# matteosantama/dantzig

Hardware: AMD Instinct MI355X
Metric: simplex_iterations_per_sec (higher is better)
Workload: dtype f64

## Files before the change

dantzig_amd/_build.py:

```python
from __future__ import annotations

import os
import shutil
import subprocess
from concurrent.futures import ThreadPoolExecutor

HERE = os.path.dirname(os.path.abspath(__file__))
CSRC = os.path.join(HERE, "csrc")
OBJ = os.path.join(HERE, "_obj")
LIB = os.path.join(HERE, "libdantzig_amd.so")
ARCH = "gfx950"
SOURCES = ["engine.hip", "k_vector.hip", "k_price.hip", "k_strict.hip", "k_fast.hip", "k_chain.hip", "k_sparse.hip", "k_refactor.hip", "k_rowshard.hip", "k_drift.hip", "k_batch.hip", "k_batch_fast.hip",
           "k_mip.hip", "k_duals.hip", "k_ranging.hip", "k_rays.hip", "model.cpp", "mip.cpp", "lpgen.cpp"]
FLAGS = ["-O3", "-std=c++17", "-fPIC", "-ffp-contract=off", "-fno-fast-math", "-Wall",
         "-Wno-unused-result", "-Wno-unused-value"]


def _hipcc() -> str:
    exe = shutil.which("hipcc") or "/opt/rocm/bin/hipcc"
    if not os.path.exists(exe):
        raise RuntimeError("hipcc not found: dantzig_amd needs the ROCm toolchain to build")
    return exe


def _newest(paths) -> float:
    return max(os.path.getmtime(p) for p in paths)


def _deps():
    hdrs = [os.path.join(CSRC, "common.h"), os.path.join(CSRC, "k_price_kernels.h"),
            os.path.join(CSRC, "fast_decide.h"), os.path.join(CSRC, "fast_rows.h"),
            os.path.join(CSRC, "chain_barrier.h"), os.path.join(CSRC, "batch_strict.h"),
            os.path.join(CSRC, "batch_host.h"),
            os.path.join(CSRC, "mip_internal.h"), os.path.join(CSRC, "duals.h"), os.path.join(CSRC, "ranging.h"), os.path.join(CSRC, "rays.h"),
            os.path.join(os.path.dirname(HERE), "include", "dantzig_amd.h")]
    return hdrs


def _compile(src: str) -> str:
    path = os.path.join(CSRC, src)
    obj = os.path.join(OBJ, src + ".o")
    if os.path.exists(obj) and os.path.getmtime(obj) >= _newest([path] + _deps()):
        return obj
    cmd = [_hipcc(), f"--offload-arch={ARCH}", *FLAGS, "-c", path, "-o", obj]
    if src.endswith(".cpp"):
        cmd.insert(1, "-x")
        cmd.insert(2, "c++")
        cmd = [c for c in cmd if not c.startswith("--offload-arch")]
    subprocess.check_call(cmd)
    return obj


def build(force: bool = False, verbose: bool = False) -> str:
    os.makedirs(OBJ, exist_ok=True)
    if force:
# ... 17 lines not shown
```

dantzig_amd/csrc/chain_barrier.h:

```cpp
#pragma once
#include "common.h"

#define CH_THREADS 512
#define CH_AGCAP DZG_CHAIN_AGCAP
#define CH_GROUPS 8
#define CH_PAD 16

__device__ __forceinline__ void st_sc1(double *p, double v)
{
    __hip_atomic_store(p, v, __ATOMIC_RELAXED, __HIP_MEMORY_SCOPE_AGENT);
}
__device__ __forceinline__ void st_sc1(int *p, int v)
{
    __hip_atomic_store(p, v, __ATOMIC_RELAXED, __HIP_MEMORY_SCOPE_AGENT);
}
__device__ __forceinline__ double ld_sc1(const double *p)
{
    return __hip_atomic_load(p, __ATOMIC_RELAXED, __HIP_MEMORY_SCOPE_AGENT);
}
__device__ __forceinline__ int ld_sc1(const int *p)
{
    return __hip_atomic_load(p, __ATOMIC_RELAXED, __HIP_MEMORY_SCOPE_AGENT);
}

#define CH_BAR_WORDS (CH_PAD * (2 + CH_GROUPS))
#define CH_POISON (1ull << 62)

__device__ __forceinline__ bool chain_barrier(DzgCtl *ctl, unsigned long long *bar,
                                              unsigned long long &gen)
{
    __shared__ int s_bar_ok;
    __syncthreads();
    if (threadIdx.x == 0) {
        gen += 1;
        const unsigned grp = blockIdx.x % CH_GROUPS;
        const unsigned long long members = (gridDim.x - grp + CH_GROUPS - 1) / CH_GROUPS;
        const unsigned long long ngroups = gridDim.x < CH_GROUPS ? gridDim.x : CH_GROUPS;
        const unsigned long long target = gen * ngroups;
        unsigned long long *frozen = bar + (size_t)CH_PAD * (1 + CH_GROUPS);
        __builtin_amdgcn_s_waitcnt(0);
        const unsigned long long old = __hip_atomic_fetch_add(
            bar + (size_t)CH_PAD * (1 + grp), 1ull, __ATOMIC_RELAXED, __HIP_MEMORY_SCOPE_AGENT);
        int ok = -1;
        unsigned long long val = 0;
        if (old + 1 == gen * members) {
            val = __hip_atomic_fetch_add(bar, 1ull, __ATOMIC_RELAXED, __HIP_MEMORY_SCOPE_AGENT);
            if (val & CH_POISON) ok = 0;
            val = 0;
        }
        if (ok < 0) {
            int spin = 0;
            for (; spin < (1 << 24); ++spin) {
                val = __hip_atomic_load(bar, __ATOMIC_RELAXED, __HIP_MEMORY_SCOPE_AGENT);
                if (val >= target) break;
                __builtin_amdgcn_s_sleep(1);
            }
            if (spin == (1 << 24)) {
                val = __hip_atomic_fetch_or(bar, CH_POISON, __ATOMIC_RELAXED, __HIP_MEMORY_SCOPE_AGENT);
                if (!(val & CH_POISON)) {
                    __hip_atomic_store(frozen, val + 1, __ATOMIC_RELAXED, __HIP_MEMORY_SCOPE_AGENT);
                    ok = val >= target ? 1 : 0;
                }
            } else if (!(val & CH_POISON)) {
                ok = 1;
            }
        }
        if (ok < 0) {
            unsigned long long f = 0;
            for (int spin = 0; spin < (1 << 22) && f == 0; ++spin) {
                f = __hip_atomic_load(frozen, __ATOMIC_RELAXED, __HIP_MEMORY_SCOPE_AGENT);
                if (f == 0) __builtin_amdgcn_s_sleep(1);
            }
            ok = (f != 0 && f - 1 >= target) ? 1 : 0;
        }
        if (!ok) {
            __hip_atomic_store(&ctl->status, (int)DZG_PANIC, __ATOMIC_RELAXED, __HIP_MEMORY_SCOPE_AGENT);
            __hip_atomic_store(&ctl->bar_timeout, 1, __ATOMIC_RELAXED, __HIP_MEMORY_SCOPE_AGENT);
        }
        s_bar_ok = ok;
    }
    __syncthreads();
    return s_bar_ok != 0;
}
```

dantzig_amd/csrc/common.h:

```cpp
#pragma once

#include <hip/hip_runtime.h>
#include <stdint.h>

#include "../../include/dantzig_amd.h"

#define DZG_WAVE 64

struct DzgCtl {
    int status;
    int kind;
    long long iter;
    long long iter_stop;
    int enter_pos;
    int leave_pos;
    int enter_var;
    int leave_var;
    double mu;
    double t, s, tbar, sbar;
    long long nb_struct;
    double price_bytes;
    int lu_mu;
    int lu_pivot_zero;
    int ncompact;
// ... 476 lines not shown
    const double *A;
    int csc;
    const long long *cptr;
    const int *ridx;
    const double *cval;
    const int *var_col;
    int *basis, *nonbasis;
    double *x, *xbar, *z, *zbar;
    double *dx, *dz, *v, *acol;
    DzgCtl *ctl;
    int *log_kind, *log_enter, *log_leave;
    double *log_mu;
    long long log_cap;
    double *binv;
    long long ldb;
    int *drow;
    int *dslot;
    double *U;
    double *W;
    long long ldw;
    double *Wc;
    double *ag;
    double *beta;
    double *beta_part;
    int beta_split;
    int *plist;
    int *pslot;
    int *pcode;
    int *cpos;
    double *fpx_r, *fpz_r, *rx_r, *rz_r;
    int *fpx_k, *fpz_k, *rx_k, *rz_k;
    double *fpx_h, *fpz_h, *rx_h, *rz_h;
    double *log_margin;
    int *bcode, *nbcode;
    int spb;
    const long long *rptr;
    const int *cidx;
    const double *rval;
    int *sslot;
    int *spos;
    int *bslot;
    int *rowpos;
    int *bcnt;
    int *bcol;
    double *bval;
    double *dxs;
    int *acol_code;
    int *lcnt;
// ... 129 lines not shown
```

dantzig_amd/csrc/engine.hip:

```cpp
#include <dlfcn.h>

#include <chrono>
#include <cstdio>
#include <cstdlib>
#include <cstring>
#include <limits>
#include <string>
#include <utility>
#include <algorithm>
#include <vector>

#include "common.h"
#include "duals.h"
#include "ranging.h"
#include "rays.h"

static thread_local std::string g_err;

static int fail(int code, const std::string &msg)
{
    g_err = msg;
    return code;
}

// ... 330 lines not shown
    if (o.stream) {
        s->st = (hipStream_t)o.stream;
        s->own_stream = false;
    } else {
        HIP_OK(hipStreamCreate(&s->st));
    }
    HIP_OK(hipHostMalloc((void **)&s->h_ctl, sizeof(DzgCtl)));

    DzgDev &d = s->d;
    const int m = (int)lp->m, n = (int)lp->n, ns = (int)lp->n_struct, q = n - m;
    d.m = m; d.n = n; d.ns = ns; d.q = q;
    d.lda = ((long long)m + 15) / 16 * 16 + (m >= 2048 ? 272 : 0);
    if (d.lda == 0) d.lda = 16;
    d.eps = o.epsilon;
    d.ftran_variant = -1;
    if (const char *fv = std::getenv("DZG_FTRAN_VARIANT")) d.ftran_variant = std::atoi(fv);
    {
        const double kk = 384e6 / (8.0 * (double)(lp->m > 0 ? lp->m : 1));
        d.ftran_nt_k = kk > 2e9 ? 2000000000 : (int)kk;
        if (d.ftran_nt_k < 513) d.ftran_nt_k = 513;
    }
    d.beta_split = 1;
    if (const char *bs = std::getenv("DZG_CHAIN_BETA_SPLIT")) d.beta_split = bs[0] != '0';
    d.fold_k = 0x7fffffff;
    if (const char *fk = std::getenv("DZG_CHAIN_FOLD_K")) d.fold_k = std::atoi(fk);
    d.world = o.world > 1 ? o.world : 1;
    d.rank = d.world > 1 ? o.rank : 0;
    d.col0 = 0;
    d.col1 = ns;
    if (d.world > 1) {
        if (o.rank < 0 || o.rank >= o.world || o.col_begin < 0 || o.col_end > ns ||
            o.col_begin > o.col_end)
            return fail(DZG_E_ARG, "opts.rank / col_begin / col_end");
        d.col0 = (int)o.col_begin;
        d.col1 = (int)o.col_end;
    }
    const int nloc = d.col1 - d.col0;
    d.repl = (d.world > 1 && o.replicate_matrix && lp->a) ? 1 : 0;
    d.xstride = d.repl ? 8 : 8 + ((long long)m + 7) / 8 * 8;
    const double *a_host = !lp->a ? nullptr
                           : (o.a_is_block && d.world > 1) ? lp->a
                                                           : lp->a + (size_t)d.col0 * (size_t)lp->lda;

    d.csc = (ns > 0 && !lp->a) ? 1 : 0;
    d.rs = 0;
    d.rs_r0 = 0;
// ... 229 lines not shown
            HIP_OK(hipMemcpyAsync(s->dr_c, lp->c, sizeof(double) * n, hipMemcpyHostToDevice, s->st));
            HIP_OK(hipMemcpyAsync(s->dr_cb, cbar.data(), sizeof(double) * n, hipMemcpyHostToDevice, s->st));
            HIP_OK(hipStreamSynchronize(s->st));
        }
        {
            const long long base = ((long long)m + 15) / 16 * 16;
            long long pad = ((160 - base % 512) % 512 + 512) % 512;
            if (pad < 32) pad += 512;
            if (const char *e = std::getenv("DZG_LDB_PAD")) pad = std::atoi(e) / 16 * 16;
            d.ldb = base + pad;
        }
        d.ldw = ((long long)m + 15) / 16 * 16 + 64;
        {
            const size_t rows_kept = d.rs ? (size_t)(d.rs_r1 - d.rs_r0) : (size_t)m;
            double *binv_alloc = nullptr;
            TRY(dev_alloc(s, &binv_alloc, (rows_kept ? rows_kept : 1) * (size_t)d.ldb));
            d.binv = binv_alloc - (d.rs ? (long long)d.rs_r0 * d.ldb : 0);
        }
        TRY(dev_alloc(s, &d.drow, (size_t)m)); TRY(dev_alloc(s, &d.dslot, (size_t)m));
        TRY(dev_alloc(s, &d.U, (size_t)d.ldw * DZG_RMAX));
        TRY(dev_alloc(s, &d.W, (size_t)d.ldw * DZG_RMAX));
        TRY(dev_alloc(s, &d.Wc, (size_t)d.ldw * DZG_RMAX));
        TRY(dev_alloc(s, &d.ag, (size_t)m + 2)); TRY(dev_alloc(s, &d.beta, (size_t)DZG_RMAX));
        TRY(dev_alloc(s, &d.beta_part, (size_t)4 * DZG_RMAX));
        TRY(dev_alloc(s, &d.plist, (size_t)q)); TRY(dev_alloc(s, &d.pslot, (size_t)q));
        TRY(dev_alloc(s, &d.bcode, (size_t)m)); TRY(dev_alloc(s, &d.nbcode, (size_t)q));
        TRY(dev_alloc(s, &d.pcode, (size_t)q));
        if (!d.csc) TRY(dev_alloc(s, &d.cpos, (size_t)(d.col1 > d.col0 ? d.col1 - d.col0 : 1)));
        const size_t np = 4096;
        TRY(dev_alloc(s, &d.fpx_r, np)); TRY(dev_alloc(s, &d.fpz_r, np));
        TRY(dev_alloc(s, &d.rx_r, np)); TRY(dev_alloc(s, &d.rz_r, np));
        TRY(dev_alloc(s, &d.fpx_k, np)); TRY(dev_alloc(s, &d.fpz_k, np));
        TRY(dev_alloc(s, &d.rx_k, np)); TRY(dev_alloc(s, &d.rz_k, np));
        TRY(dev_alloc(s, &d.fpx_h, np)); TRY(dev_alloc(s, &d.fpz_h, np));
        TRY(dev_alloc(s, &d.rx_h, np)); TRY(dev_alloc(s, &d.rz_h, np));
        if (o.refactor_interval != 0) TRY(refactor_workspace(s));
        if (d.spb && !o.seven_launches) {
            hipDeviceProp_t prop;
            HIP_OK(hipGetDeviceProperties(&prop, o.device));
            const int cus = prop.multiProcessorCount > 0 ? prop.multiProcessorCount : 1;
            const char *off = std::getenv("DZG_SP_FUSED");
            if (!(off && off[0] == '0') && (long long)dzg_sp_fused_resident_per_cu() * cus >= dzg_sp_grid(m)) {
                TRY(dev_alloc(s, &s->chain_bar, (size_t)DZG_CHAIN_BAR_WORDS));
                HIP_OK(hipMemsetAsync(s->chain_bar, 0, sizeof(unsigned long long) * DZG_CHAIN_BAR_WORDS, s->st));
            }
        }
        if (d.spb) {
// ... 529 lines not shown
    }
    default: return health_give_up(s, stop);
    }
}

static int budget_spent(dzg_solver *s, bool *spent)
{
    *spent = s->h_ctl->status == DZG_RUNNING && s->h_ctl->iter >= s->h_ctl->iter_stop;
    if (*spent) {
        int st = DZG_ITER_LIMIT;
        HIP_OK(hipMemcpy(&s->d.ctl->status, &st, sizeof(int), hipMemcpyHostToDevice));
        s->h_ctl->status = st;
    }
    return 0;
}

static int chain_recover(dzg_solver *s)
{
    DzgCtl *h = s->h_ctl;
    s->chain_fallbacks += 1;
    s->chain_retry_iter = s->chain_fallbacks >= 3 ? std::numeric_limits<long long>::max()
                                                  : h->iter + 64ll * s->opts.poll_interval;
    HIP_OK(hipMemsetAsync(s->chain_bar, 0, sizeof(unsigned long long) * DZG_CHAIN_BAR_WORDS, s->st));
    h->status = DZG_RUNNING;
    h->bar_timeout = 0;
    h->bar_gen = 0;
    HIP_OK(hipMemcpyAsync(&s->d.ctl->status, &h->status, sizeof(int), hipMemcpyHostToDevice, s->st));
    HIP_OK(hipMemcpyAsync(&s->d.ctl->bar_timeout, &h->bar_timeout, sizeof(int), hipMemcpyHostToDevice, s->st));
    HIP_OK(hipMemcpyAsync(&s->d.ctl->bar_gen, &h->bar_gen, sizeof(unsigned long long), hipMemcpyHostToDevice, s->st));
    HIP_OK(hipStreamSynchronize(s->st));
    return 0;
}

static int run_fast(dzg_solver *s)
{
    for (;;) {
        bool spent = false;
        TRY(budget_spent(s, &spent));
        if (spent) break;
        if (s->opts.refactor_interval > 0 && s->since_refactor >= s->opts.refactor_interval)
            TRY(refactor_now(s));
        const long long before = s->h_ctl->iter;
        const int batch = batch_size(s);
        s->since_flush = s->h_ctl->neta;
        s->d.price_cols_hint = (int)s->h_ctl->nb_struct + batch;
        const int k_bound = (int)s->h_ctl->ncompact + batch;
// ... 102 lines not shown

static int set_budget(dzg_solver *s, int64_t max_new_iters)
{
    if (s->d.repl && s->cols_present != s->d.ns)
        return fail(DZG_E_ARG, "replicate_matrix: " + std::to_string(s->d.ns - s->cols_present) +
                               " structural columns have not been uploaded (dzg_solver_upload_columns)");
    s->d.k_hint = s->d.k_lo_hint = 0;
    if (s->pending_refactor && !partitioned(s)) TRY(refactor_now(s));
    if (s->pending_refactor && !s->comm && !s->in_lockstep)
        return fail(DZG_E_ARG, "a non-slack starting basis of a partitioned column-sharded solver is "
                               "factorised by dzg_shard_run / dzg_shard_run_lockstep (the ranks exchange "
                               "their basic columns): a host that drives the phases itself starts from "
                               "the slack basis or uses replicate_matrix");
    TRY(read_ctl(s));
    DzgCtl *h = s->h_ctl;
    s->since_flush = h->neta;
    if (h->status != DZG_RUNNING && h->status != DZG_ITER_LIMIT && h->status != DZG_NEAR_TIE)
        return h->status;
    long long stop = s->opts.max_iter;
    if (max_new_iters > 0 && h->iter + max_new_iters < stop) stop = h->iter + max_new_iters;
    if (h->status == DZG_ITER_LIMIT && h->iter >= s->opts.max_iter) return h->status;
    if (h->status == DZG_NEAR_TIE) {
        h->tie_skip_iter = h->iter;
        HIP_OK(hipMemcpyAsync(&s->d.ctl->tie_skip_iter, &h->tie_skip_iter, sizeof(long long),
                              hipMemcpyHostToDevice, s->st));
    }
    h->status = DZG_RUNNING;
    h->iter_stop = stop;
    HIP_OK(hipMemcpyAsync(&s->d.ctl->status, &h->status, sizeof(int), hipMemcpyHostToDevice, s->st));
    HIP_OK(hipMemcpyAsync(&s->d.ctl->iter_stop, &h->iter_stop, sizeof(long long), hipMemcpyHostToDevice, s->st));
    HIP_OK(hipStreamSynchronize(s->st));
    return DZG_RUNNING;
}

extern "C" int dzg_solver_set_budget(dzg_solver *s, int64_t max_new_iters)
{
    if (!s) return fail(DZG_E_ARG, "solver is NULL");
    HIP_OK(hipSetDevice(s->opts.device));
    return set_budget(s, max_new_iters);
}

extern "C" int dzg_solver_set_profile(dzg_solver *s, int32_t mask)
{
    if (!s) return fail(DZG_E_ARG, "solver is NULL");
    if (mask != 0 && s->ev.empty())
        return fail(DZG_E_ARG, "kernel timing needs opts.profile != 0 at creation (it reserves the events)");
// ... 1515 lines not shown
```

dantzig_amd/csrc/k_chain.hip:

```cpp
#include <chrono>
#include "common.h"
#include "fast_decide.h"
#include "fast_rows.h"

#include "chain_barrier.h"


#define CH_NW (CH_THREADS / 64)
#define CH_MAXP 16

template <bool NARROW>
__device__ __forceinline__ bool chain_wide(int k)
{
    if constexpr (NARROW)
        return false;
    else
        return k > 512;
}
template <bool NOFOLD>
__device__ __forceinline__ int chain_fold_on(int fold)
{
    if constexpr (NOFOLD)
        return 0;
    else
// ... 140 lines not shown
                                               const double *__restrict__ a,
                                               const int *__restrict__ drow, int dr0, int dr1)
{
    const int k2 = (k + 1) & ~1, tid = threadIdx.x;
    const int rr = -1 - code;
    if (tid < k2) s_ag[tid] = tid < k ? (code < 0 ? (dr0 == rr ? 1.0 : 0.0) : a[dr0]) : 0.0;
    if (tid + CH_THREADS < k2)
        s_ag[tid + CH_THREADS] = tid + CH_THREADS < k ? (code < 0 ? (dr1 == rr ? 1.0 : 0.0) : a[dr1]) : 0.0;
    for (int c = tid + 2 * CH_THREADS; c < k2; c += CH_THREADS)
        s_ag[c] = c < k ? (code < 0 ? (drow[c] == rr ? 1.0 : 0.0) : a[drow[c]]) : 0.0;
}

template <bool SHARD>
__device__ __forceinline__ const double *chain_col(const DzgDev &d, int code,
                                                   const double *__restrict__ xrecv, int w_rec)
{
    if (code < 0) return nullptr;
    if (SHARD && d.xstride > 8) return xrecv + (long long)w_rec * d.xstride + 8;
    return d.A + (long long)(code - d.col0) * d.lda;
}

#define CH_BETA_WAVE 3
__device__ __forceinline__ void chain_beta_item(const DzgDev &d, int item, int code,
                                                const double *__restrict__ a)
{
    const int t = item >> 2, w = item & 3;
    const double *wt = d.W + (long long)t * d.ldw;
    double s;
    if (code < 0) {
        if (w != 0) return;
        s = wt[-1 - code];
    } else {
        s = fast_beta_wave(wt, a, d.m, w);
    }
    if ((threadIdx.x & 63) == 0) st_sc1(d.beta_part + item, s);
}
__device__ __forceinline__ void chain_beta(const DzgDev &d, int neta, int code,
                                           const double *__restrict__ a)
{
    const int wave = threadIdx.x >> 6;
    if (!d.beta_split) {
        for (int b = blockIdx.x; b < neta; b += gridDim.x)
            if (wave < 4) chain_beta_item(d, 4 * b + wave, code, a);
        return;
    }
    int turn = CH_BETA_WAVE;
    for (int item = blockIdx.x; item < 4 * neta; item += gridDim.x) {
        if (wave == turn) chain_beta_item(d, item, code, a);
        turn = turn + 1 < CH_NW ? turn + 1 : 0;
    }
}
__device__ __forceinline__ void chain_beta_published()
{
    __builtin_amdgcn_s_waitcnt(0);
}
__device__ __forceinline__ void chain_beta_fetch(const DzgDev &d, int neta, int code, double *s_beta)
{
    const int tid = threadIdx.x;
    if (tid < 4 * R_) {
        const double s0 = tid < 4 * neta ? ld_sc1(d.beta_part + tid) : 0.0;
        const double s1 = __shfl_down(s0, 1, DZG_WAVE);
        const double s2 = __shfl_down(s0, 2, DZG_WAVE);
        const double s3 = __shfl_down(s0, 3, DZG_WAVE);
        const int t = tid >> 2;
        if ((tid & 3) == 0) s_beta[t] = t < neta ? (code < 0 ? s0 : fast_beta_fold(s0, s1, s2, s3)) : 0.0;
    }
}

template <int LPR, int MAXP>
__device__ __forceinline__ void chain_dot_head(const DzgDev &d, int r0, int r1, int k,
                                               const double *s_ag, double (&accs)[MAXP])
{
    constexpr int RPW = 64 / LPR;
    const int lane = threadIdx.x & 63, wave = threadIdx.x >> 6;
    const int sub = lane % LPR, grp = lane / LPR;
    const int k2 = (k + 1) & ~1;
    const int variant = d.ftran_variant >= 0 ? d.ftran_variant : (k >= d.ftran_nt_k ? 2 : 0);
    if (LPR == 64 && variant == 1) {
#pragma unroll
        for (int pass = 0; pass < MAXP; ++pass) {
            const int i = r0 + (pass * CH_NW + wave) * RPW + grp;
            accs[pass] = fast_gemv_row_head<LPR, 1>(i < r1 ? i : d.m, d.m, k2, d.binv, d.ldb, s_ag, sub);
        }
        return;
    }
    if (LPR == 64 && variant == 2) {
#pragma unroll
        for (int pass = 0; pass < MAXP; ++pass) {
// ... 24 lines not shown
        if (pass < npass) {
            const int i = r0 + (pass * CH_NW + wave) * RPW + grp;
            const int ii = i < r1 ? i : d.m;
            const double acc = fast_gemv_row_tail<LPR>(accs[pass], ii, d.m, neta, d.U, d.ldw, s_beta, sub);
            if (ii < d.m && sub == 0) s_dx[i - r0] = acc;
        }
    }
    for (int pass = MAXP; pass < npass; ++pass) {
        const int i = r0 + (pass * CH_NW + wave) * RPW + grp;
        const int ii = i < r1 ? i : d.m;
        const double acc = fast_gemv_row<LPR>(ii, d.m, k2, neta, d.binv, d.ldb, s_ag, d.U, d.ldw, s_beta, sub);
        if (ii < d.m && sub == 0) s_dx[i - r0] = acc;
    }
}

template <bool SHARD, int MAXP, bool NARROW>
__global__ __launch_bounds__(CH_THREADS) void k_chain_pre(const DzgDev d, unsigned long long *bar,
                                                          unsigned long long *dbg,
                                                          const double *__restrict__ xrecv)
{
    __shared__ double s_ag[CH_AGCAP];
    __shared__ double s_beta[R_], s_dx[CH_THREADS], s_up[R_];
    __shared__ ChainSlots s_c;
    ChainStamps ts;
    ts.start(dbg);
    DzgCtl *ctl = d.ctl;
    const int tid = threadIdx.x, lane = tid & 63, wave = tid >> 6;
    const int m = d.m, nwg = (int)gridDim.x;
    const bool lead = blockIdx.x == 0 && tid == 0;
    ChainSpec sp;
    if (wave == 0 && !SHARD)
        chain_spec_load(sp, d.fpz_r, d.fpz_k, d.fpz_h, lane);
    else if (wave == 1)
        chain_spec_load(sp, d.fpx_r, d.fpx_k, d.fpx_h, lane);
    DzgCand2 cj_rec = dzg_cand2_none();
    int w_rec = -1;
    if (SHARD) w_rec = shard_merge(xrecv, d.xstride, d.world, cj_rec);
    int r0, r1;
    chain_rows(m, r0, r1);
    const int row = r0 + tid;
    const bool has_row = row < r1;
    int dslot_i = -1, bcode_i = 0;
    double x_i = 0.0, xbar_i = 0.0;
    if (has_row) {
        dslot_i = d.dslot[row];
        bcode_i = d.bcode[row];
// ... 27 lines not shown
    if (k > CH_AGCAP || c.fp_count > 256 || (NARROW && k > 512)) {
        if (lead) ctl->status = DZG_PANIC;
        return;
    }
    if (lead) {
        ctl->neta_cur = neta;
        ctl->k_cur = k;
    }
    int p;
    if (kind == DZG_STEP_PRIMAL) {
        const int epos = cj.k;
        const int code = d.nbcode[epos];
        double zr = 0.0, zbr = 0.0;
        if (lead) {
            zr = d.z[epos];
            zbr = d.zbar[epos];
        }
        const double *a = chain_col<SHARD>(d, code, xrecv, w_rec);
        const bool has_unit = has_row && bcode_i < 0;
        double unit_i = 0.0;
        if (has_unit) unit_i = code >= 0 ? a[-1 - bcode_i] : (code == bcode_i ? 1.0 : 0.0);
        int edslot = -1;
        if (lead && code < 0) edslot = d.dslot[-1 - code];
        chain_stage_ag(s_ag, k, code, a, d.drow, dr0, dr1);
        chain_beta(d, neta, code, a);
        ts.mark(slot);
        if (lead) {
            ctl->enter_code = code;
            ctl->zr = zr;
            ctl->zbar_r = zbr;
            ctl->enter_dslot = edslot;
            if (SHARD) ctl->enter_src = w_rec;
        }
        __syncthreads();
        double accs[MAXP];
        if (chain_wide<NARROW>(k))
            chain_dot_head<64>(d, r0, r1, k, s_ag, accs);
        else
            chain_dot_head<16>(d, r0, r1, k, s_ag, accs);
        chain_beta_published();
        ts.mark(slot);
        if (!chain_barrier(ctl, bar, gen)) return;
        ts.mark(slot);
        chain_beta_fetch(d, neta, code, s_beta);
        __syncthreads();
        if (chain_wide<NARROW>(k))
            chain_dot_tail<64>(d, r0, r1, k, neta, s_ag, s_beta, accs, s_dx);
        else
            chain_dot_tail<16>(d, r0, r1, k, neta, s_ag, s_beta, accs, s_dx);
        __syncthreads();
        DzgCand2 best = dzg_cand2_none();
        if (has_row) {
            double dxi = s_dx[tid];
            if (has_unit) dxi += unit_i;
            d.dx[row] = dxi;
            const double scaled = mu * xbar_i;
            const double den = x_i + scaled;
            DzgCand2 cnd;
            cnd.r = dzg_div(dxi, den);
            cnd.k = row;
            cnd.h = -__builtin_inf();
            if (cnd.r > 0.0) best = dzg_better2(best, cnd);
            if (dzg_noise_zero(den, x_i, scaled, c.tau)) best.h = __builtin_inf();
        }
        ts.pin(best);
        const unsigned long long t_rowbest = ts.now();
        best = chain_best(best, r1 - r0);
        ts.pin(best);
        ts.site(DZG_SITE_PRE_ROWBEST, t_rowbest);
        if (tid == 0) {
            st_sc1(d.rx_r + blockIdx.x, best.r);
            st_sc1(d.rx_k + blockIdx.x, best.k);
            st_sc1(d.rx_h + blockIdx.x, best.h);
        }
        ts.mark(slot);
        if (!chain_barrier(ctl, bar, gen)) return;
        ts.mark(slot);
        const unsigned long long t_sc1 = ts.now();
        if (wave == 0) {
            const DzgCand2 w = chain_reduce_sc1(d.rx_r, d.rx_k, d.rx_h, nwg, lane);
            if (lane == 0) chain_put(s_c, 0, w);
        }
        __syncthreads();
        DzgCand2 cw = chain_get(s_c, 0);
        ts.pin(cw);
        ts.site(DZG_SITE_PRE_SC1, t_sc1);
        if (!fast_ratio_outcome(ctl, c, lead, cw, DZG_UNBOUNDED)) {
            if (lead) ctl->bar_gen = gen;
            return;
        }
        p = cw.k;
        if (lead) ctl->leave_pos = p;
        ts.mark(slot);
    } else {
        p = ci.k;
    }
    const int lcode = d.bcode[p];
    double xp = 0.0, xbp = 0.0;
    if (lead) {
// ... 35 lines not shown
    int gg = 0;
    for (; gg + 8 <= G; gg += 8) {
        double t[8];
#pragma unroll
        for (int e = 0; e < 8; ++e) t[e] = src[(long long)(gg + e) * d.ldt];
#pragma unroll
        for (int e = 0; e < 8; ++e) sum = sum + t[e];
    }
    for (; gg < G; ++gg) sum = sum + src[(long long)gg * d.ldt];
    return -sum;
}

template <bool SHARD, int MAXP, bool NARROW, bool NOFOLD>
__global__ __launch_bounds__(CH_THREADS) void k_chain_post(const DzgDev d, unsigned long long *bar,
                                                           const DzgPivotArgs pa, int only_partials,
                                                           int nrz, unsigned long long *dbg,
                                                           const double *__restrict__ xrecv, int fold_arg)
{
    const int fold = chain_fold_on<NOFOLD>(fold_arg);
    __shared__ double s_ag[CH_AGCAP];
    __shared__ double s_beta[R_], s_dx[CH_THREADS];
    __shared__ double s_dxp;
    __shared__ ChainSlots s_c;
    ChainStamps ts;
    ts.start(only_partials ? nullptr : dbg);
    const unsigned long long t_books = (dbg && !only_partials && blockIdx.x == 0 && threadIdx.x == CH_THREADS - 64)
                                           ? __builtin_amdgcn_s_memrealtime()
                                           : 0ull;
    int slot = 2;
    DzgCtl *ctl = d.ctl;
    const int tid = threadIdx.x, lane = tid & 63, wave = tid >> 6;
    const int m = d.m, q = d.q;
    const bool lead = blockIdx.x == 0 && tid == 0;
    DzgCand2 mine = dzg_cand2_none();
    ChainSpec sp;
    const bool one_wave = chain_one_wave<NOFOLD>(nrz);
    if (SHARD || fold) {
    } else if (!only_partials && one_wave) {
        if (wave == 0) chain_spec_load(sp, d.rz_r, d.rz_k, d.rz_h, lane);
    } else if (!only_partials) {
#pragma unroll
        for (int j = 0; j < 4; ++j) {
            const int i = tid + CH_THREADS * j;
            DzgCand2 o;
            o.r = d.rz_r[i];
            o.k = d.rz_k[i];
// ... 15 lines not shown
    const bool has_row = row < r1, has_col = col < q1;
    double x_i = 0.0, xbar_i = 0.0, v_i = 0.0, dx_i = 0.0, z_k = 0.0, zbar_k = 0.0, dz_k = 0.0;
    int bcode_i = 0, nbcode_k = -1;
    if (has_row) {
        x_i = d.x[row];
        xbar_i = d.xbar[row];
        if (!only_partials) {
            v_i = d.v[row];
            dx_i = d.dx[row];
            bcode_i = d.bcode[row];
        }
    }
    if (has_col) {
        z_k = d.z[col];
        zbar_k = d.zbar[col];
        if (!only_partials && !fold) dz_k = d.dz[col];
        if (SHARD || fold) nbcode_k = d.nbcode[col];
    }
    DzgCtl c = *ctl;
    if (c.status != DZG_RUNNING) return;
    unsigned long long gen = c.bar_gen;
    int p = 0, r = 0, teta = 0, wzero = -1, del_ce = -1, del_last = -1, app_col = -1, new_code_r = -1;
    double t = 0.0, s = 0.0, tbar = 0.0, sbar = 0.0, rdxp = 0.0, tau = c.tau;
    if (!only_partials) {
        const int neta = c.neta_cur, k = c.k_cur, kind = c.kind;
        const int ci = c.leave_code;
        const double xp = c.xp, xbp = c.xbp;
        p = c.leave_pos;
        int cj, edslot;
        double zr, zbr, dzr, dxp;
        int G = (k + 1 + DZG_PR_BATCH - 1) / DZG_PR_BATCH;
        G = G > DZG_PR_GMAX ? DZG_PR_GMAX : G;
        if (!SHARD && fold) {
            const int ncols = q1 - q0;
            int *s_code = reinterpret_cast<int *>(s_dx);
            if (has_col) s_code[tid] = nbcode_k;
            __syncthreads();
            if ((long long)ncols * G <= CH_AGCAP) {
                for (int idx = tid; idx < ncols * G; idx += CH_THREADS) {
                    const int g = idx / ncols, pl = idx - g * ncols;
                    const int code = s_code[pl];
                    s_ag[idx] = code >= 0 ? d.ppart[(long long)g * d.ldt + (code - d.col0)] : 0.0;
                }
                __syncthreads();
                if (has_col) {
                    if (nbcode_k < 0) {
// ... 66 lines not shown
                cj = (int)rec[5];
                zr = rec[2];
                zbr = rec[3];
                dzr = rec[4];
                if (lead) {
                    ctl->enter_src = w_rec;
                    ctl->zr = zr;
                    ctl->zbar_r = zbr;
                    ctl->dz_r = dzr;
                    ctl->use_record = 1;
                }
            } else {
                cj = d.nbcode[r];
                zr = d.z[r];
                zbr = d.zbar[r];
                dzr = fold ? chain_fold_dz(d, cj, G) : d.dz[r];
            }
            const double *a = chain_col<SHARD>(d, cj, xrecv, w_rec);
            edslot = cj < 0 ? d.dslot[-1 - cj] : -1;
            const bool has_unit = has_row && bcode_i < 0;
            double unit_i = 0.0, unit_p = 0.0;
            if (has_unit) unit_i = cj >= 0 ? a[-1 - bcode_i] : (cj == bcode_i ? 1.0 : 0.0);
            if (ci < 0) unit_p = cj >= 0 ? a[-1 - ci] : (cj == ci ? 1.0 : 0.0);
            chain_stage_ag(s_ag, k, cj, a, d.drow, dr0, dr1);
            chain_beta(d, neta, cj, a);
            ts.mark(slot);
            if (lead) {
                ctl->enter_pos = r;
                ctl->enter_code = cj;
            }
            c.enter_pos = r;
            c.enter_code = cj;
            __syncthreads();
            const int k2 = (k + 1) & ~1;
            double accs[MAXP], accp;
            if (chain_wide<NARROW>(k)) {
                chain_dot_head<64>(d, r0, r1, k, s_ag, accs);
                accp = fast_gemv_row_head<64>(wave == CH_NW - 1 ? p : m, m, k2, d.binv, d.ldb, s_ag, lane);
            } else {
                chain_dot_head<16>(d, r0, r1, k, s_ag, accs);
                accp = fast_gemv_row_head<16>(wave == CH_NW - 1 && lane < 16 ? p : m, m, k2, d.binv, d.ldb, s_ag,
                                              lane % 16);
            }
            chain_beta_published();
            ts.mark(slot);
            if (!chain_barrier(ctl, bar, gen)) return;
            ts.mark(slot);
            chain_beta_fetch(d, neta, cj, s_beta);
            __syncthreads();
            if (chain_wide<NARROW>(k)) {
                chain_dot_tail<64>(d, r0, r1, k, neta, s_ag, s_beta, accs, s_dx);
                if (wave == CH_NW - 1) {
                    const double acc = fast_gemv_row_tail<64>(accp, p, m, neta, d.U, d.ldw, s_beta, lane);
                    if (lane == 0) s_dxp = ci < 0 ? acc + unit_p : acc;
                }
            } else {
                chain_dot_tail<16>(d, r0, r1, k, neta, s_ag, s_beta, accs, s_dx);
                if (wave == CH_NW - 1) {
                    const double acc = fast_gemv_row_tail<16>(accp, lane < 16 ? p : m, m, neta, d.U, d.ldw,
                                                              s_beta, lane % 16);
                    if (lane == 0) s_dxp = ci < 0 ? acc + unit_p : acc;
                }
            }
            __syncthreads();
            dxp = s_dxp;
            if (has_row) {
                dx_i = s_dx[tid];
                if (has_unit) dx_i += unit_i;
                d.dx[row] = dx_i;
            }
            ts.mark(slot);
        } else {
            r = c.enter_pos;
            cj = c.enter_code;
            zr = c.zr;
            zbr = c.zbar_r;
            dzr = (!SHARD && fold) ? chain_fold_dz(d, cj, G) : d.dz[r];
            if (SHARD) {
                int w_rec = -1;
                for (int rk = 0; rk < d.world && w_rec < 0; ++rk)
                    if ((int)xrecv[(long long)rk * d.xstride + 1] == r) w_rec = rk;
                if (w_rec < 0) {
                    if (lead) ctl->status = DZG_PANIC;
                    return;
                }
                const double *rec = xrecv + (long long)w_rec * d.xstride;
                zr = rec[2];
                zbr = rec[3];
                dzr = rec[4];
                if (lead) {
                    ctl->zr = zr;
                    ctl->zbar_r = zbr;
                    ctl->dz_r = dzr;
                    ctl->use_record = 1;
                }
            }
            edslot = c.enter_dslot;
            dxp = d.dx[p];
            ts.mark(slot);
        }
        const DzgPivotScalars ps = fast_pivot_scalars(xp, xbp, dxp, zr, zbr, dzr, neta, c.max_pivot_err);
        const bool appended = ci < 0, deleted = cj < 0;
        new_code_r = ci;
        if (blockIdx.x == 0 && wave == CH_NW - 1) {
            c.neta = neta;
            c.ncompact = k;
            fast_pivot_books_s(ctl, c, pa, ps, 1);
            if (t_books && kind == DZG_STEP_DUAL && lane == 0) {
                __builtin_amdgcn_s_waitcnt(0);
                dbg[16 * DZG_SITE_SLOT + DZG_SITE_BOOKS] += __builtin_amdgcn_s_memrealtime() - t_books;
                dbg[16 * (DZG_SITE_SLOT + 1) + DZG_SITE_BOOKS] += 1;
            }
        }
        if (!ps.ok) {
            if (lead && gen != c.bar_gen) ctl->bar_gen = gen;
            return;
        }
        if (deleted) {
            del_last = k + (appended ? 1 : 0) - 1;
            del_ce = edslot;
        }
        if (appended) app_col = k;
        if (lead && gen != c.bar_gen) ctl->bar_gen = gen;
        t = ps.t;
// ... 285 lines not shown
```

Baseline: 33910.

## Replace beta grid barrier with tagged per-slot handoff and split barrier arrive/wait

Beta partial sums are now published into tagged two-word slots, so consumers poll only the slots they need instead of waiting on a full grid barrier before fetching beta. In the dual step the barrier is split into arrive and a deferred wait, letting pivot scalar computation overlap the barrier, and the dx store is moved after the wait. The aim is to remove one global barrier per iteration from the chain kernel's critical path. In exchange it adds per-slot polling, a fallback path that reverts to the barrier when a slot arrives late, and extra memsets of the slot buffer on restarts.

```diff
diff --git a/dantzig_amd/_build.py b/dantzig_amd/_build.py
--- a/dantzig_amd/_build.py
+++ b/dantzig_amd/_build.py
@@ -30,7 +30,8 @@
 def _deps():
     hdrs = [os.path.join(CSRC, "common.h"), os.path.join(CSRC, "k_price_kernels.h"),
             os.path.join(CSRC, "fast_decide.h"), os.path.join(CSRC, "fast_rows.h"),
-            os.path.join(CSRC, "chain_barrier.h"), os.path.join(CSRC, "batch_strict.h"),
+            os.path.join(CSRC, "chain_barrier.h"), os.path.join(CSRC, "chain_protocol.h"),
+            os.path.join(CSRC, "batch_strict.h"),
             os.path.join(CSRC, "batch_host.h"),
             os.path.join(CSRC, "mip_internal.h"), os.path.join(CSRC, "duals.h"), os.path.join(CSRC, "ranging.h"), os.path.join(CSRC, "rays.h"),
             os.path.join(os.path.dirname(HERE), "include", "dantzig_amd.h")]
diff --git a/dantzig_amd/csrc/chain_barrier.h b/dantzig_amd/csrc/chain_barrier.h
--- a/dantzig_amd/csrc/chain_barrier.h
+++ b/dantzig_amd/csrc/chain_barrier.h
@@ -1,10 +1,9 @@
 #pragma once
 #include "common.h"
+#include "chain_protocol.h"
 
 #define CH_THREADS 512
 #define CH_AGCAP DZG_CHAIN_AGCAP
-#define CH_GROUPS 8
-#define CH_PAD 16
 
 __device__ __forceinline__ void st_sc1(double *p, double v)
 {
@@ -23,56 +22,22 @@
     return __hip_atomic_load(p, __ATOMIC_RELAXED, __HIP_MEMORY_SCOPE_AGENT);
 }
 
-#define CH_BAR_WORDS (CH_PAD * (2 + CH_GROUPS))
-#define CH_POISON (1ull << 62)
-
-__device__ __forceinline__ bool chain_barrier(DzgCtl *ctl, unsigned long long *bar,
-                                              unsigned long long &gen)
+__device__ __forceinline__ void chain_barrier_arrive(unsigned long long *bar, unsigned long long &gen,
+                                                     ChainTicket &tk)
 {
-    __shared__ int s_bar_ok;
     __syncthreads();
     if (threadIdx.x == 0) {
         gen += 1;
-        const unsigned grp = blockIdx.x % CH_GROUPS;
-        const unsigned long long members = (gridDim.x - grp + CH_GROUPS - 1) / CH_GROUPS;
-        const unsigned long long ngroups = gridDim.x < CH_GROUPS ? gridDim.x : CH_GROUPS;
-        const unsigned long long target = gen * ngroups;
-        unsigned long long *frozen = bar + (size_t)CH_PAD * (1 + CH_GROUPS);
         __builtin_amdgcn_s_waitcnt(0);
-        const unsigned long long old = __hip_atomic_fetch_add(
-            bar + (size_t)CH_PAD * (1 + grp), 1ull, __ATOMIC_RELAXED, __HIP_MEMORY_SCOPE_AGENT);
-        int ok = -1;
-        unsigned long long val = 0;
-        if (old + 1 == gen * members) {
-            val = __hip_atomic_fetch_add(bar, 1ull, __ATOMIC_RELAXED, __HIP_MEMORY_SCOPE_AGENT);
-            if (val & CH_POISON) ok = 0;
-            val = 0;
-        }
-        if (ok < 0) {
-            int spin = 0;
-            for (; spin < (1 << 24); ++spin) {
-                val = __hip_atomic_load(bar, __ATOMIC_RELAXED, __HIP_MEMORY_SCOPE_AGENT);
-                if (val >= target) break;
-                __builtin_amdgcn_s_sleep(1);
-            }
-            if (spin == (1 << 24)) {
-                val = __hip_atomic_fetch_or(bar, CH_POISON, __ATOMIC_RELAXED, __HIP_MEMORY_SCOPE_AGENT);
-                if (!(val & CH_POISON)) {
-                    __hip_atomic_store(frozen, val + 1, __ATOMIC_RELAXED, __HIP_MEMORY_SCOPE_AGENT);
-                    ok = val >= target ? 1 : 0;
-                }
-            } else if (!(val & CH_POISON)) {
-                ok = 1;
-            }
-        }
-        if (ok < 0) {
-            unsigned long long f = 0;
-            for (int spin = 0; spin < (1 << 22) && f == 0; ++spin) {
-                f = __hip_atomic_load(frozen, __ATOMIC_RELAXED, __HIP_MEMORY_SCOPE_AGENT);
-                if (f == 0) __builtin_amdgcn_s_sleep(1);
-            }
-            ok = (f != 0 && f - 1 >= target) ? 1 : 0;
-        }
+        chain_arrive0(bar, gen, blockIdx.x, gridDim.x, tk);
+    }
+}
+__device__ __forceinline__ bool chain_barrier_wait(DzgCtl *ctl, unsigned long long *bar, const ChainTicket &tk,
+                                                   bool give_up = false)
+{
+    __shared__ int s_bar_ok;
+    if (threadIdx.x == 0) {
+        const int ok = chain_wait0(bar, tk, give_up);
         if (!ok) {
             __hip_atomic_store(&ctl->status, (int)DZG_PANIC, __ATOMIC_RELAXED, __HIP_MEMORY_SCOPE_AGENT);
             __hip_atomic_store(&ctl->bar_timeout, 1, __ATOMIC_RELAXED, __HIP_MEMORY_SCOPE_AGENT);
@@ -82,3 +47,18 @@
     __syncthreads();
     return s_bar_ok != 0;
 }
+__device__ __forceinline__ bool chain_barrier(DzgCtl *ctl, unsigned long long *bar,
+                                              unsigned long long &gen, bool absent = false)
+{
+    ChainTicket tk;
+    if (!absent) {
+        chain_barrier_arrive(bar, gen, tk);
+    } else {
+        __syncthreads();
+        if (threadIdx.x == 0) {
+            gen += 1;
+            chain_absent0(gen, gridDim.x, tk);
+        }
+    }
+    return chain_barrier_wait(ctl, bar, tk, absent) && !absent;
+}
diff --git a/dantzig_amd/csrc/chain_protocol.h b/dantzig_amd/csrc/chain_protocol.h
--- /dev/null
+++ b/dantzig_amd/csrc/chain_protocol.h
@@ -0,0 +1,155 @@
+#pragma once
+#include <stddef.h>
+#include <stdint.h>
+
+#ifdef __HIPCC__
+#define CHP_FN __device__ __forceinline__
+#define CHP_LOAD(p) __hip_atomic_load((p), __ATOMIC_RELAXED, __HIP_MEMORY_SCOPE_AGENT)
+#define CHP_STORE(p, v) __hip_atomic_store((p), (v), __ATOMIC_RELAXED, __HIP_MEMORY_SCOPE_AGENT)
+#define CHP_FETCH_ADD(p, v) __hip_atomic_fetch_add((p), (v), __ATOMIC_RELAXED, __HIP_MEMORY_SCOPE_AGENT)
+#define CHP_FETCH_OR(p, v) __hip_atomic_fetch_or((p), (v), __ATOMIC_RELAXED, __HIP_MEMORY_SCOPE_AGENT)
+#define CHP_SLEEP() __builtin_amdgcn_s_sleep(1)
+#define CHP_POLLS (1 << 24)
+#define CHP_FROZEN_POLLS (1 << 22)
+#define CHP_NOUNROLL _Pragma("nounroll")
+#else
+#define CHP_NOUNROLL
+#define CHP_FN static inline
+#define CHP_LOAD(p) __atomic_load_n((p), __ATOMIC_ACQUIRE)
+#define CHP_STORE(p, v) __atomic_store_n((p), (v), __ATOMIC_RELEASE)
+#define CHP_FETCH_ADD(p, v) __atomic_fetch_add((p), (v), __ATOMIC_ACQ_REL)
+#define CHP_FETCH_OR(p, v) __atomic_fetch_or((p), (v), __ATOMIC_ACQ_REL)
+#ifndef CHP_SLEEP
+#define CHP_SLEEP() ((void)0)
+#endif
+#ifndef CHP_POLLS
+#define CHP_POLLS (1 << 24)
+#endif
+#ifndef CHP_FROZEN_POLLS
+#define CHP_FROZEN_POLLS (1 << 22)
+#endif
+#endif
+
+#define CH_GROUPS 8
+#define CH_PAD 16
+#define CH_BAR_WORDS (CH_PAD * (2 + CH_GROUPS))
+#define CH_POISON (1ull << 62)
+
+struct ChainTicket {
+    unsigned long long target;
+    unsigned long long seen;
+    int ok;
+};
+
+CHP_FN void chain_arrive0(unsigned long long *bar, unsigned long long gen, unsigned block, unsigned grid,
+                          ChainTicket &tk)
+{
+    const unsigned grp = block % CH_GROUPS;
+    const unsigned long long members = (grid - grp + CH_GROUPS - 1) / CH_GROUPS;
+    const unsigned long long ngroups = grid < CH_GROUPS ? grid : CH_GROUPS;
+    tk.target = gen * ngroups;
+    tk.seen = 0;
+    tk.ok = -1;
+    const unsigned long long old = CHP_FETCH_ADD(bar + (size_t)CH_PAD * (1 + grp), 1ull);
+    if (old + 1 == gen * members) {
+        const unsigned long long val = CHP_FETCH_ADD(bar, 1ull);
+        if (val & CH_POISON) tk.ok = 0;
+    }
+}
+
+CHP_FN void chain_absent0(unsigned long long gen, unsigned grid, ChainTicket &tk)
+{
+    tk.target = gen * (grid < CH_GROUPS ? grid : CH_GROUPS);
+    tk.seen = 0;
+    tk.ok = -1;
+}
+
+CHP_FN void chain_peek0(const unsigned long long *bar, ChainTicket &tk)
+{
+    if (tk.ok < 0) tk.seen = CHP_LOAD(bar);
+}
+
+CHP_FN int chain_wait0(unsigned long long *bar, const ChainTicket &tk, bool give_up)
+{
+    unsigned long long *frozen = bar + (size_t)CH_PAD * (1 + CH_GROUPS);
+    const unsigned long long target = tk.target;
+    int ok = tk.ok;
+    if (ok < 0) {
+        unsigned long long val = tk.seen;
+        bool gave_up = give_up;
+        if (!give_up && val < target) {
+            int spin = 0;
+            CHP_NOUNROLL
+            for (; spin < CHP_POLLS; ++spin) {
+                val = CHP_LOAD(bar);
+                if (val >= target) break;
+                CHP_SLEEP();
+            }
+            gave_up = spin == CHP_POLLS;
+        }
+        if (gave_up) {
+            val = CHP_FETCH_OR(bar, CH_POISON);
+            if (!(val & CH_POISON)) {
+                CHP_STORE(frozen, val + 1);
+                ok = val >= target ? 1 : 0;
+            }
+        } else if (!(val & CH_POISON)) {
+            ok = 1;
+        }
+    }
+    if (ok < 0) {
+        unsigned long long f = 0;
+        CHP_NOUNROLL
+        for (int spin = 0; spin < CHP_FROZEN_POLLS && f == 0; ++spin) {
+            f = CHP_LOAD(frozen);
+            if (f == 0) CHP_SLEEP();
+        }
+        ok = (f != 0 && f - 1 >= target) ? 1 : 0;
+    }
+    return ok;
+}
+
+CHP_FN uint32_t chain_tag(long long iter)
+{
+    unsigned long long x = (unsigned long long)iter;
+    x = (x & 0xffffffffull) + (x >> 32);
+    x = (x & 0xffffffffull) + (x >> 32);
+    x = (x & 0xffffffffull) + (x >> 32);
+    if (x == 0xffffffffull) x = 0;
+    return (uint32_t)x + 1u;
+}
+
+CHP_FN void chain_slot_put(unsigned long long *slot, double v, uint32_t tag)
+{
+    unsigned long long b;
+    __builtin_memcpy(&b, &v, sizeof(b));
+    CHP_STORE(slot, (b & 0xffffffff00000000ull) | tag);
+    CHP_STORE(slot + 1, (b << 32) | tag);
+}
+
+CHP_FN bool chain_slot_ready(unsigned long long g0, unsigned long long g1, uint32_t tag)
+{
+    return (uint32_t)g0 == tag && (uint32_t)g1 == tag;
+}
+
+CHP_FN double chain_slot_value(unsigned long long g0, unsigned long long g1)
+{
+    const unsigned long long b = (g0 & 0xffffffff00000000ull) | (g1 >> 32);
+    double v;
+    __builtin_memcpy(&v, &b, sizeof(v));
+    return v;
+}
+
+CHP_FN bool chain_slot_wait(const unsigned long long *slot, uint32_t tag, double *v)
+{
+    CHP_NOUNROLL
+    for (int spin = 0; spin < CHP_POLLS; ++spin) {
+        const unsigned long long g0 = CHP_LOAD(slot), g1 = CHP_LOAD(slot + 1);
+        if (chain_slot_ready(g0, g1, tag)) {
+            *v = chain_slot_value(g0, g1);
+            return true;
+        }
+        CHP_SLEEP();
+    }
+    return false;
+}
diff --git a/dantzig_amd/csrc/common.h b/dantzig_amd/csrc/common.h
--- a/dantzig_amd/csrc/common.h
+++ b/dantzig_amd/csrc/common.h
@@ -522,8 +522,9 @@
     double *Wc;
     double *ag;
     double *beta;
-    double *beta_part;
+    unsigned long long *beta_part;
     int beta_split;
+    int beta_handoff;
     int *plist;
     int *pslot;
     int *pcode;
diff --git a/dantzig_amd/csrc/engine.hip b/dantzig_amd/csrc/engine.hip
--- a/dantzig_amd/csrc/engine.hip
+++ b/dantzig_amd/csrc/engine.hip
@@ -376,6 +376,8 @@
     }
     d.beta_split = 1;
     if (const char *bs = std::getenv("DZG_CHAIN_BETA_SPLIT")) d.beta_split = bs[0] != '0';
+    d.beta_handoff = 1;
+    if (const char *bh = std::getenv("DZG_CHAIN_BETA_HANDOFF")) d.beta_handoff = bh[0] != '0';
     d.fold_k = 0x7fffffff;
     if (const char *fk = std::getenv("DZG_CHAIN_FOLD_K")) d.fold_k = std::atoi(fk);
     d.world = o.world > 1 ? o.world : 1;
@@ -651,7 +653,8 @@
         TRY(dev_alloc(s, &d.W, (size_t)d.ldw * DZG_RMAX));
         TRY(dev_alloc(s, &d.Wc, (size_t)d.ldw * DZG_RMAX));
         TRY(dev_alloc(s, &d.ag, (size_t)m + 2)); TRY(dev_alloc(s, &d.beta, (size_t)DZG_RMAX));
-        TRY(dev_alloc(s, &d.beta_part, (size_t)4 * DZG_RMAX));
+        TRY(dev_alloc(s, &d.beta_part, (size_t)8 * DZG_RMAX));
+        HIP_OK(hipMemsetAsync(d.beta_part, 0, sizeof(unsigned long long) * 8 * DZG_RMAX, s->st));
         TRY(dev_alloc(s, &d.plist, (size_t)q)); TRY(dev_alloc(s, &d.pslot, (size_t)q));
         TRY(dev_alloc(s, &d.bcode, (size_t)m)); TRY(dev_alloc(s, &d.nbcode, (size_t)q));
         TRY(dev_alloc(s, &d.pcode, (size_t)q));
@@ -1227,6 +1230,7 @@
     s->chain_retry_iter = s->chain_fallbacks >= 3 ? std::numeric_limits<long long>::max()
                                                   : h->iter + 64ll * s->opts.poll_interval;
     HIP_OK(hipMemsetAsync(s->chain_bar, 0, sizeof(unsigned long long) * DZG_CHAIN_BAR_WORDS, s->st));
+    HIP_OK(hipMemsetAsync(s->d.beta_part, 0, sizeof(unsigned long long) * 8 * DZG_RMAX, s->st));
     h->status = DZG_RUNNING;
     h->bar_timeout = 0;
     h->bar_gen = 0;
@@ -1375,6 +1379,8 @@
     if (h->status == DZG_ITER_LIMIT && h->iter >= s->opts.max_iter) return h->status;
     if (h->status == DZG_NEAR_TIE) {
         h->tie_skip_iter = h->iter;
+        if (s->d.beta_part)
+            HIP_OK(hipMemsetAsync(s->d.beta_part, 0, sizeof(unsigned long long) * 8 * DZG_RMAX, s->st));
         HIP_OK(hipMemcpyAsync(&s->d.ctl->tie_skip_iter, &h->tie_skip_iter, sizeof(long long),
                               hipMemcpyHostToDevice, s->st));
     }
diff --git a/dantzig_amd/csrc/k_chain.hip b/dantzig_amd/csrc/k_chain.hip
--- a/dantzig_amd/csrc/k_chain.hip
+++ b/dantzig_amd/csrc/k_chain.hip
@@ -186,7 +186,7 @@
 
 #define CH_BETA_WAVE 3
 __device__ __forceinline__ void chain_beta_item(const DzgDev &d, int item, int code,
-                                                const double *__restrict__ a)
+                                                const double *__restrict__ a, uint32_t tag)
 {
     const int t = item >> 2, w = item & 3;
     const double *wt = d.W + (long long)t * d.ldw;
@@ -197,20 +197,20 @@
     } else {
         s = fast_beta_wave(wt, a, d.m, w);
     }
-    if ((threadIdx.x & 63) == 0) st_sc1(d.beta_part + item, s);
+    if ((threadIdx.x & 63) == 0) chain_slot_put(d.beta_part + 2 * item, s, tag);
 }
 __device__ __forceinline__ void chain_beta(const DzgDev &d, int neta, int code,
-                                           const double *__restrict__ a)
+                                           const double *__restrict__ a, uint32_t tag)
 {
     const int wave = threadIdx.x >> 6;
     if (!d.beta_split) {
         for (int b = blockIdx.x; b < neta; b += gridDim.x)
-            if (wave < 4) chain_beta_item(d, 4 * b + wave, code, a);
+            if (wave < 4) chain_beta_item(d, 4 * b + wave, code, a, tag);
         return;
     }
     int turn = CH_BETA_WAVE;
     for (int item = blockIdx.x; item < 4 * neta; item += gridDim.x) {
-        if (wave == turn) chain_beta_item(d, item, code, a);
+        if (wave == turn) chain_beta_item(d, item, code, a, tag);
         turn = turn + 1 < CH_NW ? turn + 1 : 0;
     }
 }
@@ -218,16 +218,27 @@
 {
     __builtin_amdgcn_s_waitcnt(0);
 }
-__device__ __forceinline__ void chain_beta_fetch(const DzgDev &d, int neta, int code, double *s_beta)
-{
-    const int tid = threadIdx.x;
-    if (tid < 4 * R_) {
-        const double s0 = tid < 4 * neta ? ld_sc1(d.beta_part + tid) : 0.0;
+__device__ __forceinline__ void chain_beta_fetch(const DzgDev &d, int neta, int code, uint32_t tag,
+                                                 double *s_beta, int *s_late)
+{
+    static_assert(CH_THREADS >= 4 * R_ && (4 * R_) % 64 == 0, "whole waves");
+    const int tid = (int)threadIdx.x - (CH_THREADS - 4 * R_);
+    if (tid >= 0) {
+        double s0 = 0.0;
+        if (tid < 4 * neta && (code >= 0 || (tid & 3) == 0))
+            if (!chain_slot_wait(d.beta_part + 2 * tid, tag, &s0)) *s_late = 1;
         const double s1 = __shfl_down(s0, 1, DZG_WAVE);
         const double s2 = __shfl_down(s0, 2, DZG_WAVE);
         const double s3 = __shfl_down(s0, 3, DZG_WAVE);
         const int t = tid >> 2;
         if ((tid & 3) == 0) s_beta[t] = t < neta ? (code < 0 ? s0 : fast_beta_fold(s0, s1, s2, s3)) : 0.0;
+    }
+}
+__device__ __forceinline__ void chain_beta_lost(DzgCtl *ctl)
+{
+    if (threadIdx.x == 0) {
+        __hip_atomic_store(&ctl->status, (int)DZG_PANIC, __ATOMIC_RELAXED, __HIP_MEMORY_SCOPE_AGENT);
+        __hip_atomic_store(&ctl->bar_timeout, 1, __ATOMIC_RELAXED, __HIP_MEMORY_SCOPE_AGENT);
     }
 }
 
@@ -298,6 +309,7 @@
     __shared__ double s_ag[CH_AGCAP];
     __shared__ double s_beta[R_], s_dx[CH_THREADS], s_up[R_];
     __shared__ ChainSlots s_c;
+    __shared__ int s_late;
     ChainStamps ts;
     ts.start(dbg);
     DzgCtl *ctl = d.ctl;
@@ -371,8 +383,10 @@
         if (has_unit) unit_i = code >= 0 ? a[-1 - bcode_i] : (code == bcode_i ? 1.0 : 0.0);
         int edslot = -1;
         if (lead && code < 0) edslot = d.dslot[-1 - code];
+        const uint32_t tag = chain_tag(c.iter);
         chain_stage_ag(s_ag, k, code, a, d.drow, dr0, dr1);
-        chain_beta(d, neta, code, a);
+        chain_beta(d, neta, code, a, tag);
+        if (tid == 0) s_late = 0;
         ts.mark(slot);
         if (lead) {
             ctl->enter_code = code;
@@ -389,17 +403,20 @@
             chain_dot_head<16>(d, r0, r1, k, s_ag, accs);
         chain_beta_published();
         ts.mark(slot);
-        if (!chain_barrier(ctl, bar, gen)) return;
+        if (!d.beta_handoff && !chain_barrier(ctl, bar, gen)) return;
         ts.mark(slot);
-        chain_beta_fetch(d, neta, code, s_beta);
+        chain_beta_fetch(d, neta, code, tag, s_beta, &s_late);
         __syncthreads();
-        if (chain_wide<NARROW>(k))
-            chain_dot_tail<64>(d, r0, r1, k, neta, s_ag, s_beta, accs, s_dx);
-        else
-            chain_dot_tail<16>(d, r0, r1, k, neta, s_ag, s_beta, accs, s_dx);
+        const bool late = s_late != 0;
+        if (!late) {
+            if (chain_wide<NARROW>(k))
+                chain_dot_tail<64>(d, r0, r1, k, neta, s_ag, s_beta, accs, s_dx);
+            else
+                chain_dot_tail<16>(d, r0, r1, k, neta, s_ag, s_beta, accs, s_dx);
+        }
         __syncthreads();
         DzgCand2 best = dzg_cand2_none();
-        if (has_row) {
+        if (has_row && !late) {
             double dxi = s_dx[tid];
             if (has_unit) dxi += unit_i;
             d.dx[row] = dxi;
@@ -423,7 +440,7 @@
             st_sc1(d.rx_h + blockIdx.x, best.h);
         }
         ts.mark(slot);
-        if (!chain_barrier(ctl, bar, gen)) return;
+        if (!chain_barrier(ctl, bar, gen, late)) return;
         ts.mark(slot);
         const unsigned long long t_sc1 = ts.now();
         if (wave == 0) {
@@ -505,6 +522,7 @@
     __shared__ double s_beta[R_], s_dx[CH_THREADS];
     __shared__ double s_dxp;
     __shared__ ChainSlots s_c;
+    __shared__ int s_late;
     ChainStamps ts;
     ts.start(only_partials ? nullptr : dbg);
     const unsigned long long t_books = (dbg && !only_partials && blockIdx.x == 0 && threadIdx.x == CH_THREADS - 64)
@@ -566,6 +584,8 @@
     unsigned long long gen = c.bar_gen;
     int p = 0, r = 0, teta = 0, wzero = -1, del_ce = -1, del_last = -1, app_col = -1, new_code_r = -1;
     double t = 0.0, s = 0.0, tbar = 0.0, sbar = 0.0, rdxp = 0.0, tau = c.tau;
+    ChainTicket tk = {0ull, 0ull, -1};
+    bool wait_due = false;
     if (!only_partials) {
         const int neta = c.neta_cur, k = c.k_cur, kind = c.kind;
         const int ci = c.leave_code;
@@ -678,8 +698,10 @@
             double unit_i = 0.0, unit_p = 0.0;
             if (has_unit) unit_i = cj >= 0 ? a[-1 - bcode_i] : (cj == bcode_i ? 1.0 : 0.0);
             if (ci < 0) unit_p = cj >= 0 ? a[-1 - ci] : (cj == ci ? 1.0 : 0.0);
+            const uint32_t tag = chain_tag(c.iter);
             chain_stage_ag(s_ag, k, cj, a, d.drow, dr0, dr1);
-            chain_beta(d, neta, cj, a);
+            chain_beta(d, neta, cj, a, tag);
+            if (tid == 0) s_late = 0;
             ts.mark(slot);
             if (lead) {
                 ctl->enter_pos = r;
@@ -700,10 +722,25 @@
             }
             chain_beta_published();
             ts.mark(slot);
-            if (!chain_barrier(ctl, bar, gen)) return;
+            chain_barrier_arrive(bar, gen, tk);
+            wait_due = true;
             ts.mark(slot);
-            chain_beta_fetch(d, neta, cj, s_beta);
-            __syncthreads();
+            for (bool give_up = false;;) {
+                if (!d.beta_handoff || give_up) {
+                    if (!chain_barrier_wait(ctl, bar, tk, give_up)) return;
+                    wait_due = false;
+                }
+                chain_beta_fetch(d, neta, cj, tag, s_beta, &s_late);
+                __syncthreads();
+                if (!s_late) break;
+                if (!wait_due) {
+                    chain_beta_lost(ctl);
+                    return;
+                }
+                __syncthreads();
+                if (tid == 0) s_late = 0;
+                give_up = true;
+            }
             if (chain_wide<NARROW>(k)) {
                 chain_dot_tail<64>(d, r0, r1, k, neta, s_ag, s_beta, accs, s_dx);
                 if (wave == CH_NW - 1) {
@@ -718,12 +755,12 @@
                     if (lane == 0) s_dxp = ci < 0 ? acc + unit_p : acc;
                 }
             }
+            if (wait_due && tid == 0) chain_peek0(bar, tk);
             __syncthreads();
             dxp = s_dxp;
             if (has_row) {
                 dx_i = s_dx[tid];
                 if (has_unit) dx_i += unit_i;
-                d.dx[row] = dx_i;
             }
             ts.mark(slot);
         } else {
@@ -756,6 +793,8 @@
             ts.mark(slot);
         }
         const DzgPivotScalars ps = fast_pivot_scalars(xp, xbp, dxp, zr, zbr, dzr, neta, c.max_pivot_err);
+        if (wait_due && !chain_barrier_wait(ctl, bar, tk)) return;
+        if (kind == DZG_STEP_DUAL && has_row) d.dx[row] = dx_i;
         const bool appended = ci < 0, deleted = cj < 0;
         new_code_r = ci;
         if (blockIdx.x == 0 && wave == CH_NW - 1) {
```

After: 33760. Within noise of the previous version (-0.4%).
